# pmorenoz/HetMOGP

Hardware: AMD Instinct MI355X
Metric: ELBO-steps/sec (one step = ELBO + all parameter gradients) (higher is better)
Workload: dtype f64

## Files before the change

__graft_entry__.py:

```python
import os
import subprocess
import sys

ROOT = os.path.dirname(os.path.abspath(__file__))
CSRC = os.path.join(ROOT, "hetmogp_amd", "csrc")


def build():
    jobs = str(min(8, os.cpu_count() or 1))
    subprocess.run(["make", "-C", CSRC, "-j", jobs], check=True)
    probes = os.path.join(ROOT, "tools", "probes")
    os.makedirs(os.path.join(probes, "build"), exist_ok=True)
    for name in ("probe_mfma", "probe_coissue", "probe_gemm8", "probe_gemm16", "probe_gemm_abl", "probe_i8"):
        r = subprocess.run(["/opt/rocm/bin/hipcc", "--offload-arch=gfx950", "-O3", "-Wno-unused-value",
                            os.path.join(probes, name + ".hip"), "-o", os.path.join(probes, "build", name)], check=False)
        if r.returncode != 0:
            print("build(): diagnostic probe %s did not compile (not part of libhetmogp_hip.so)" % name, file=sys.stderr)
    if ROOT not in sys.path:
        sys.path.insert(0, ROOT)
    import hetmogp_amd
    from hetmogp_amd import _lib
    assert os.path.exists(_lib.LIB_PATH)


def smoke():
    if ROOT not in sys.path:
        sys.path.insert(0, ROOT)
    import numpy as np
    from hetmogp_amd.engine import Engine
    from hetmogp_amd.synthetic import make_case
    from oracle import svmogp_oracle as so

    specs = [("Gaussian", {"sigma": 0.5}), ("Bernoulli", {}), ("Poisson", {}), ("Gamma", {})]
    for M, N in ((64, 2000), (128, 20000)):
        prm, X, Y = make_case(specs, [N] * 4, M=M, Q=3, P=1, seed=7)
        prob = so.make_problem(specs, 3, M, 1)
        want = so.elbo_grad_fused(prm, prob, X, Y)
        e = Engine(specs, 3, M, 1, device=0)
        e.set_data(X, Y)
        out = e.elbo_grad(**prm)
        worst = 0.0
        for k in ("elbo", "g_m_u", "g_L_u", "g_variance", "g_lengthscale", "g_W", "g_kappa", "g_Z"):
            a, b = np.asarray(out[k], float), np.asarray(want[k], float)
            err = float(np.max(np.abs(a - b)) / (np.max(np.abs(b)) + 1e-300))
            worst = max(worst, err)
            assert err < 1e-8, (M, k, err)
        ms, _ = e.timings()
        print("smoke OK (M=%d, N_t=%d): ELBO %.6f (oracle %.6f), worst relative error %.2e, %.2f ms on device" %
              (M, N, out["elbo"], want["elbo"], worst, ms["total"]))
        e.close()
    g = np.load(os.path.join(ROOT, "tests", "golden", "lad_h_mix_M128_ladder.npz"))
    prm, prob, X, Y, bs = so.load_case(g)
    e = Engine(prob["specs"], prob["Q"], prob["M"], prob["P"], device=0, strict_qf=True)
    e.set_data(X, Y)
    out = e.elbo_grad(batch_scale=bs, **prm)
    assert out["rungs"] == [int(r) for r in g["rungs"]], out["rungs"]
    worst = 0.0
    for k in ("elbo", "g_m_u", "g_L_u", "g_variance", "g_lengthscale", "g_W", "g_kappa", "g_Z"):
        a, b = np.asarray(out[k], float).ravel(), np.asarray(g[k], float).ravel()
        ex = float(np.max(np.abs(a - b) / (1e-5 * np.abs(b) + 1e-9 * np.max(np.abs(b)))))
        worst = max(worst, ex)
        assert ex <= 1.0, ("strict mode vs reference run", k, ex)
    print("smoke OK (strict q(f), M=128, jitter rung %s as in the reference run): worst element-wise excess over 1e-5 criterion %.3f" %
          (out["rungs"], worst))
    from hetmogp_amd import _lib
    oe = e.elbo_grad(batch_scale=bs, group_mask=_lib.GROUP_QU, **prm)
    worst_e = 0.0
    for k in ("elbo", "g_m_u", "g_L_u"):
        a, b = np.asarray(oe[k], float).ravel(), np.asarray(g[k], float).ravel()
        ex = float(np.max(np.abs(a - b) / (1e-5 * np.abs(b) + 1e-9 * np.max(np.abs(b)))))
        worst_e = max(worst_e, ex)
        assert ex <= 1.0, ("strict E-step (one-solve form) vs reference run", k, ex)
    print("smoke OK (strict E-step, one-solve form): worst element-wise excess %.3f" % worst_e)
    e.close()


if __name__ == "__main__":
    build()
    if len(sys.argv) > 1 and sys.argv[1] == "smoke":
        smoke()
```

hetmogp_amd/csrc/gemm_rowpass.hip:

```cpp
#include <cstdlib>

#include "common.h"

namespace {

constexpr int BM = 128, BN = 128, BK = 16, W = 8, NT = W * 64;
constexpr int KM_LD = 144, RM_LD = 18, TILE_DOUBLES = BK * KM_LD;
constexpr int NB = 2, WN = 32, NWN = 4;

struct Tile {
  double a[2][TILE_DOUBLES];
  double b[2][TILE_DOUBLES];
};

__device__ __forceinline__ int diag_wm(int w) { return (0x4B >> w) & 1; }
__device__ __forceinline__ int diag_wn(int w) { return (0x7E84 >> (2 * w)) & 3; }

template <int ROLE, bool FOLD = false>
__device__ __forceinline__ void rowpass_tile(const GemmArgs& g, int tiles_n, int ti, int tj, int split, Tile& lds, double* epi_a,
                                             int* hwinfo = nullptr) {
  const int batch = blockIdx.z;
  const int M = g.M, N = g.N, K = g.K;
  const int i0 = ti * BM, j0 = tj * BN;
  if (i0 >= M || j0 >= N) return;
  int wlo = 0;
  if (ROLE == 1 && g.b_tri > 0) wlo = j0;
  const int ksteps = (K - wlo + BK - 1) / BK;
  const int per = (ksteps + g.ksplit - 1) / g.ksplit;
  const int kbeg = wlo + split * per * BK;
  const int kend = min(K, kbeg + per * BK);

  const double* __restrict__ A = g.A + (long long)batch * g.sA;
  const double* __restrict__ B = g.B + (long long)batch * g.sB;
  const double* __restrict__ S = (ROLE == 2) ? g.kscale + (long long)batch * g.sS : nullptr;
  double* __restrict__ C = g.C + (long long)batch * g.sC + (long long)split * g.sSplit;
  double* fs_part = (ROLE == 1 && g.fs_part) ? g.fs_part + (long long)batch * g.fs_sPart : nullptr;

  const int t = threadIdx.x, lane = t & 63, w = __builtin_amdgcn_readfirstlane(t >> 6);
  const int lr = lane & 15, lk = lane >> 4;
  int wm = w >> 2, wn = w & 3;
  if (FOLD && w >= 4) wn = 3 - wn;
  const int klive = FOLD ? j0 + 32 * wn : 0;
  unsigned sub = 0xFFu;
  const bool diag = ROLE == 2 && ti == tj && g.lower_only;
  if (diag && hwinfo) {
    if (lane == 0) {
      const unsigned hw = __builtin_amdgcn_s_getreg(4 | (0 << 6) | (31 << 11));
      hwinfo[w] = (int)((hw >> 4) & 3u);
      if (w == 0) hwinfo[8] = (int)((hw >> 1) & 1u);
    }
  }
  constexpr bool SWAP = (ROLE == 1);
  const int blr = SWAP ? 4 * (lr & 3) + (lr >> 2) : lr;

  f64x4 acc[4][NB];
#pragma unroll
  for (int a = 0; a < 4; ++a)
#pragma unroll
    for (int b = 0; b < NB; ++b) acc[a][b] = f64x4{0.0, 0.0, 0.0, 0.0};

  const int ar = t >> 2, ak = (t & 3) * 4, bk = t >> 5, bc = (t & 31) * 2;
  const double* pa;
  const double* pb;
  if (ROLE == 1) {
    pa = A + (long long)min(i0 + ar, M - 1) * g.lda + ak;
    pb = B + (long long)bk * g.ldb + j0 + bc;
  } else {
    pa = A + i0 + bc;
    pb = B + j0 + bc;
  }
  double ra[4], rb[4], ks = 1.0;
  auto load = [&](int k0) {
    if (ROLE == 1) {
      const f64x2 x0 = *reinterpret_cast<const f64x2*>(pa + k0), x1 = *reinterpret_cast<const f64x2*>(pa + k0 + 2);
      ra[0] = x0.x, ra[1] = x0.y, ra[2] = x1.x, ra[3] = x1.y;
      const double* q = pb + (long long)k0 * g.ldb;
      const f64x2 y0 = *reinterpret_cast<const f64x2*>(q), y1 = *reinterpret_cast<const f64x2*>(q + 64);
      rb[0] = y0.x, rb[1] = y0.y, rb[2] = y1.x, rb[3] = y1.y;
    } else {
      const int row = k0 + bk;
      const long long off = (long long)min(row, K - 1) * g.lda;
      const f64x2 x0 = *reinterpret_cast<const f64x2*>(pa + off), x1 = *reinterpret_cast<const f64x2*>(pa + off + 64);
      ra[0] = x0.x, ra[1] = x0.y, ra[2] = x1.x, ra[3] = x1.y;
      const f64x2 y0 = *reinterpret_cast<const f64x2*>(pb + off), y1 = *reinterpret_cast<const f64x2*>(pb + off + 64);
      rb[0] = y0.x, rb[1] = y0.y, rb[2] = y1.x, rb[3] = y1.y;
      ks = (row < kend) ? S[row] : 0.0;
    }
  };
  auto stage = [&](int buf) {
    if (ROLE == 1) {
      double* sa = &lds.a[buf][ar * RM_LD + ak];
      *reinterpret_cast<f64x2*>(sa) = f64x2{ra[0], ra[1]};
      *reinterpret_cast<f64x2*>(sa + 2) = f64x2{ra[2], ra[3]};
    } else {
      double* sa = &lds.a[buf][bk * KM_LD + bc];
      *reinterpret_cast<f64x2*>(sa) = f64x2{ra[0], ra[1]};
      *reinterpret_cast<f64x2*>(sa + 64) = f64x2{ra[2], ra[3]};
#pragma unroll
      for (int i = 0; i < 4; ++i) rb[i] *= ks;
    }
    double* sb = &lds.b[buf][bk * KM_LD + bc];
    *reinterpret_cast<f64x2*>(sb) = f64x2{rb[0], rb[1]};
    *reinterpret_cast<f64x2*>(sb + 64) = f64x2{rb[2], rb[3]};
  };
  double fa[2][4], fb[2][NB];
  auto frag = [&](int buf, int kk, int s) {
    const double* fpa = (ROLE == 1) ? &lds.a[buf][(wm * 64 + lr) * RM_LD + kk * 4 + lk] : &lds.a[buf][(kk * 4 + lk) * KM_LD + wm * 64 + lr];
    const double* fpb = &lds.b[buf][(kk * 4 + lk) * KM_LD + wn * WN + blr];
#pragma unroll
    for (int i = 0; i < 4; ++i) fa[s][i] = fpa[i * 16 * (ROLE == 1 ? RM_LD : 1)];
#pragma unroll
    for (int i = 0; i < NB; ++i) fb[s][i] = fpb[i * 16];
  };
  auto mm8 = [&](int s) {
#pragma unroll
    for (int a = 0; a < 4; ++a)
#pragma unroll
      for (int b = 0; b < NB; ++b) {
        if (ROLE == 2 && !((sub >> (a * NB + b)) & 1u)) continue;
        acc[a][b] = SWAP ? __builtin_amdgcn_mfma_f64_16x16x4f64(fb[s][b], fa[s][a], acc[a][b], 0, 0, 0)
                         : __builtin_amdgcn_mfma_f64_16x16x4f64(fa[s][a], fb[s][b], acc[a][b], 0, 0, 0);
      }
  };

  int cur = 0;
  if (kbeg < kend) {
    load(kbeg);
    stage(0);
    if (kbeg + BK < kend) load(kbeg + BK);
  }
  __syncthreads();
  if (diag) {
    int role = w;
    if (hwinfo) {
      bool ok = true;
      unsigned seen = 0;
#pragma unroll
      for (int i = 0; i < 4; ++i) {
        ok = ok && hwinfo[i] == hwinfo[i + 4];
        seen |= 1u << hwinfo[i];
      }
      if (ok && seen == 0xFu) role = ((hwinfo[w] + 2 * hwinfo[8]) & 3) + (w & 4);
    }
    role = __builtin_amdgcn_readfirstlane(role);
    wm = diag_wm(role), wn = diag_wn(role);
    sub = 0;
#pragma unroll
    for (int a = 0; a < 4; ++a)
#pragma unroll
      for (int b = 0; b < NB; ++b)
        if (wn * NB + b <= wm * 4 + a) sub |= 1u << (a * NB + b);
  }
  const bool live = ROLE == 1 || sub != 0;
  if (ROLE == 2) {
    for (int k0 = kbeg; k0 < kend; k0 += BK) {
      if (k0 + BK < kend) stage(cur ^ 1);
      if (k0 + 2 * BK < kend) load(k0 + 2 * BK);
      if (live) {
#pragma unroll
        for (int kk = 0; kk < BK / 4; ++kk) {
          frag(cur, kk, 0);
          mm8(0);
        }
      }
      __syncthreads();
      cur ^= 1;
    }
  }
  if (ROLE == 1 && kbeg < kend && (!FOLD || kbeg >= klive)) frag(0, 0, 0);
#define HM_SB __builtin_amdgcn_sched_barrier(0)
  for (int k0 = kbeg; ROLE == 1 && k0 < kend; k0 += BK) {
    const bool more = k0 + BK < kend;
    const bool lv = !FOLD || k0 >= klive;
    if (lv) {
      frag(cur, 1, 1);
      HM_SB;
      mm8(0);
      HM_SB;
    }
    if (more) stage(cur ^ 1);
    if (k0 + 2 * BK < kend) load(k0 + 2 * BK);
    HM_SB;
    if (lv) {
      frag(cur, 2, 0);
      HM_SB;
      mm8(1);
      HM_SB;
      frag(cur, 3, 1);
      HM_SB;
      mm8(0);
      HM_SB;
    }
    __syncthreads();
    if (more && (!FOLD || k0 + BK >= klive)) frag(cur ^ 1, 0, 0);
    if (lv) {
      HM_SB;
      mm8(1);
      HM_SB;
    }
    cur ^= 1;
  }
#undef HM_SB

  if (ROLE == 1 && fs_part && g.fs_sq) {
#pragma unroll
    for (int a = 0; a < 4; ++a) {
      double sq = 0.0;
#pragma unroll
      for (int b = 0; b < NB; ++b)
#pragma unroll
        for (int r = 0; r < 4; ++r) sq = fma(acc[a][b][r], acc[a][b][r], sq);
      sq += __shfl_xor(sq, 16, 64);
      sq += __shfl_xor(sq, 32, 64);
      const int rl = wm * 64 + a * 16 + lr;
      if (lk == 0 && i0 + rl < M) fs_part[((long long)NWN * tiles_n + NWN * tj + wn) * M + (i0 + rl)] = sq;
    }
    if (!g.store_c) return;
  } else if (ROLE == 1 && fs_part) {
    constexpr int NCH = 2 * NB, WSTAGE = 2 * NCH * 128;
    double* flat = &lds.a[0][0];
    double* stg = flat + w * WSTAGE;
    static_assert(W * WSTAGE <= 4 * TILE_DOUBLES, "epilogue scratch fits the tile buffers");
    const int colq = j0 + wn * WN + 4 * lk;
    const double* __restrict__ Ke = g.fs_k ? g.fs_k + (long long)batch * g.sA : A;
    auto issue = [&](int a) {
      const int grow = min(i0 + wm * 64 + a * 16 + lr, M - 1);
      const double* src = Ke + (long long)grow * g.lda + colq;
      double* dst = stg + (a & 1) * (NCH * 128);
#pragma unroll
      for (int c = 0; c < NCH; ++c)
        __builtin_amdgcn_global_load_lds((const void __attribute__((address_space(1)))*)(src + (c >> 1) * 16 + (c & 1) * 2),
                                         (void __attribute__((address_space(3)))*)(dst + c * 128), 16, 0, 0);
    };
    issue(0);
    issue(1);
    if (t < 128) epi_a[t] = g.fs_a[(long long)batch * g.fs_sA + j0 + t];
    __syncthreads();
#pragma unroll
    for (int a = 0; a < 4; ++a) {
      if (a < 3) asm volatile("s_waitcnt vmcnt(4)" ::: "memory");
      else asm volatile("s_waitcnt vmcnt(0)" ::: "memory");
      const int rl = wm * 64 + a * 16 + lr;
      double sp = 0.0, sc = 0.0;
#pragma unroll
      for (int b = 0; b < NB; ++b) {
        const int cl = wn * WN + b * 16 + 4 * lk;
        const double* kp = stg + (a & 1) * (NCH * 128) + (2 * b) * 128 + 2 * lane;
        const f64x2 k01 = *reinterpret_cast<const f64x2*>(kp), k23 = *reinterpret_cast<const f64x2*>(kp + 128);
        const double kv[4] = {k01.x, k01.y, k23.x, k23.y};
        const f64x2 a01 = *reinterpret_cast<const f64x2*>(epi_a + cl), a23 = *reinterpret_cast<const f64x2*>(epi_a + cl + 2);
        const double av[4] = {a01.x, a01.y, a23.x, a23.y};
#pragma unroll
        for (int r = 0; r < 4; ++r) {
          sp += kv[r] * av[r];
          sc += acc[a][b][r] * kv[r];
        }
      }
#pragma unroll
      for (int o = 16; o <= 32; o <<= 1) {
        sp += __shfl_xor(sp, o, 64);
        sc += __shfl_xor(sc, o, 64);
      }
      if (lk == 0 && i0 + rl < M) {
        double* o = fs_part + ((long long)(NWN * tj + wn)) * M + (i0 + rl);
        const long long ss = (long long)NWN * tiles_n * M;
        o[0] = sp, o[ss] = sc;
      }
      if (a < 2) {
        asm volatile("" ::: "memory");
        issue(a + 2);
      }
    }
    if (!g.store_c) return;
  }
  if (SWAP) {
#pragma unroll
    for (int a = 0; a < 4; ++a) {
      const int row = i0 + wm * 64 + a * 16 + lr;
      if (row >= M) continue;
      double* crow = C + (long long)row * g.ldc + j0 + wn * WN + 4 * lk;
      if (g.c_sub) {
        const double* srow = g.c_src ? g.c_src + (long long)batch * g.sC + (long long)row * g.ldc + j0 + wn * WN + 4 * lk : crow;
#pragma unroll
        for (int b = 0; b < NB; ++b) {
          const f64x2 c01 = *reinterpret_cast<const f64x2*>(srow + b * 16), c23 = *reinterpret_cast<const f64x2*>(srow + b * 16 + 2);
          *reinterpret_cast<f64x2*>(crow + b * 16) = f64x2{c01.x - acc[a][b][0], c01.y - acc[a][b][1]};
          *reinterpret_cast<f64x2*>(crow + b * 16 + 2) = f64x2{c23.x - acc[a][b][2], c23.y - acc[a][b][3]};
        }
        continue;
      }
#pragma unroll
      for (int b = 0; b < NB; ++b) {
        *reinterpret_cast<f64x2*>(crow + b * 16) = f64x2{acc[a][b][0], acc[a][b][1]};
        *reinterpret_cast<f64x2*>(crow + b * 16 + 2) = f64x2{acc[a][b][2], acc[a][b][3]};
      }
    }
    return;
  }
#pragma unroll
  for (int a = 0; a < 4; ++a)
#pragma unroll
    for (int r = 0; r < 4; ++r) {
      double* crow = C + (long long)(i0 + wm * 64 + a * 16 + 4 * r + lk) * g.ldc + j0 + wn * WN + lr;
#pragma unroll
      for (int b = 0; b < NB; ++b)
        if ((sub >> (a * NB + b)) & 1u) crow[b * 16] = acc[a][b][r];
    }
}

template <int ROLE, bool PAIR>
__device__ __forceinline__ void rowpass_block(const GemmArgs& g, int tiles_n, int ntiles, Tile& lds, double* epi_a,
                                              int* hwinfo = nullptr) {

  int v = blockIdx.x, split = 0;
  int ti, tj;
  if (ROLE == 2 && g.lower_only) {
    const int T = tiles_n, noff = T * (T - 1) / 2, ks8 = (g.ksplit > 1) ? ((g.ksplit + 7) / 8) * 8 : 1, gx1 = noff * ks8;
    if (v < gx1) {
      int u = v;
      if (g.ksplit > 1) {
        const int xcd = v & 7, idx = v >> 3;
        split = (idx / noff) * 8 + xcd;
        u = idx % noff;
      }
      ti = (int)((sqrt(8.0 * (double)u + 1.0) + 1.0) * 0.5);
      while (ti * (ti + 1) / 2 <= u) ++ti;
      while (ti * (ti - 1) / 2 > u) --ti;
      tj = u - ti * (ti - 1) / 2;
    } else {
      const int u = v - gx1;
      split = u / T;
      ti = tj = u - split * T;
    }
    if (split >= g.ksplit) return;
  } else {
    if (g.ksplit > 1) {
      const int xcd = v & 7, idx = v >> 3;
      split = (idx / ntiles) * 8 + xcd;
      v = idx % ntiles;
      if (split >= g.ksplit) return;
    } else if ((ntiles & 7) == 0) {
      const int cpx = ntiles >> 3;
      v = (v & 7) * cpx + (v >> 3);
    }
    const int tcols = PAIR ? tiles_n / 2 : tiles_n;
    ti = v / tcols;
    tj = v - ti * tcols;
  }
  rowpass_tile<ROLE, PAIR>(g, tiles_n, ti, tj, split, lds, epi_a, hwinfo);
  if (PAIR) {
    __syncthreads();
    rowpass_tile<ROLE, PAIR>(g, tiles_n, ti, tiles_n - 1 - tj, split, lds, epi_a);
  }
}

template <int ROLE>
__global__ __launch_bounds__(NT, 4) void rowpass_gemm_kernel(GemmArgs g, int tiles_n, int ntiles) {
  __shared__ __attribute__((aligned(16))) Tile lds;
  __shared__ __attribute__((aligned(16))) double epi_a[ROLE == 1 ? 128 : 2];
  __shared__ int hwinfo[ROLE == 2 ? 16 : 1];
  rowpass_block<ROLE, false>(g, tiles_n, ntiles, lds, epi_a, ROLE == 2 ? hwinfo : nullptr);
}
__global__ __launch_bounds__(NT, 4) void rowpass_fold_pair_kernel(GemmArgs g, int tiles_n, int ntiles) {
  __shared__ __attribute__((aligned(16))) Tile lds;
  __shared__ __attribute__((aligned(16))) double epi_a[128];
  rowpass_block<1, true>(g, tiles_n, ntiles, lds, epi_a);
}

bool aligned16(const void* p) { return (((uintptr_t)p) & 15) == 0; }

}

bool gemm_rowpass_eligible(const GemmArgs& g) {
  const bool sub = g.role == 1 && g.alpha == -1.0 && g.beta == 1.0 && !g.fs_part && g.b_tri == 0 && g.store_c;
  if (g.nouter != 1 || (!sub && (g.alpha != 1.0 || g.beta != 0.0)) || g.win || g.M_last || g.N_last || g.K_last || g.a_tri) return false;
  if ((g.lda & 1) || (g.ldb & 1) || (g.ldc & 1) || !aligned16(g.A) || !aligned16(g.B) || !aligned16(g.C)) return false;
  if (g.c_src && (!sub || !aligned16(g.c_src))) return false;
  if (g.fs_k && (g.role != 1 || !g.fs_part || g.fs_sq || !aligned16(g.fs_k))) return false;
  if ((g.sA & 1) || (g.sB & 1) || (g.sC & 1) || (g.sSplit & 1)) return false;
  if (g.role == 1)
    return !g.a_kmajor && g.b_kmajor && !g.lower_only && g.ksplit == 1 && !g.kscale && g.b_tri >= 0 && (g.N % BN) == 0 &&
           (g.K % BK) == 0 && (g.K == g.N || sub) && g.K >= BK && g.M >= 1;
  if (g.role == 2)
    return g.a_kmajor && g.b_kmajor && g.kscale && g.b_tri == 0 && g.M == g.N && (g.N % BN) == 0 &&
           g.lda == g.ldb && g.K >= 1;
  return false;
}

void launch_gemm_rowpass(const GemmArgs& g_in, hipStream_t stream) {
  GemmArgs g = g_in;
  g.c_sub = (g.role == 1 && g.alpha == -1.0 && g.beta == 1.0) ? 1 : 0;
  const int tiles_m = (g.M + BM - 1) / BM, tiles_n = (g.N + BN - 1) / BN;
  const int ntiles = g.lower_only ? tiles_m * (tiles_m + 1) / 2 : tiles_m * tiles_n;
  const int gx = (g.ksplit > 1) ? ntiles * ((g.ksplit + 7) / 8) * 8 : ntiles;
  dim3 grid(gx, 1, g.nbatch);
  if (g.role == 1) {
    const int pair = (g.b_tri > 0 && g.ksplit == 1 && tiles_n >= 2 && (tiles_n & 1) == 0) ? 1 : 0;
    if (pair) {
      grid.x = tiles_m * (tiles_n / 2);
      hipLaunchKernelGGL(rowpass_fold_pair_kernel, grid, dim3(NT), 0, stream, g, tiles_n, (int)grid.x);
    } else {
      hipLaunchKernelGGL((rowpass_gemm_kernel<1>), grid, dim3(NT), 0, stream, g, tiles_n, ntiles);
    }
  } else {
    hipLaunchKernelGGL((rowpass_gemm_kernel<2>), grid, dim3(NT), 0, stream, g, tiles_n, ntiles);
  }
}

int launch_gemm_rowpass_or_general(const GemmArgs& g, hipStream_t stream) {
  const bool eligible = gemm_rowpass_eligible(g);
  if ((g.fs_sq || g.fs_k) && !eligible)
    throw HipError{hipErrorInvalidValue, "fs_sq / fs_k are features of the specialised forward kernel only", __FILE__, __LINE__};
  if (eligible) {
    launch_gemm_rowpass(g, stream);
    return NWN;
  }
  if (g.role == 1 && (g.alpha != 1.0 || g.beta != 0.0)) {
    GemmArgs h = g;
    h.role = 0;
    launch_gemm_f64(h, stream);
    return 2;
  }
  launch_gemm_f64(g, stream);
  return 2;
}
```

Before: 8.386.

## Load B fragments directly from global via buffer loads in forward rowpass GEMM

Adds a B-direct variant of the forward (role 1) rowpass GEMM. B fragments are fetched straight from global memory into registers with raw buffer loads and a two-slot ring, while only A is staged through LDS at BK=32 with a new padded layout. This removes LDS traffic and barriers for B and halves the number of k-step syncs. The variant is selected when K is a multiple of 32, there is no subtract epilogue, no triangular B, and the buffer range fits in 32 bits; otherwise the old staged kernel runs. It risks global-load latency on the MFMA critical path and less reuse of B across waves.

```diff
diff --git a/__graft_entry__.py b/__graft_entry__.py
--- a/__graft_entry__.py
+++ b/__graft_entry__.py
@@ -11,7 +11,7 @@
     subprocess.run(["make", "-C", CSRC, "-j", jobs], check=True)
     probes = os.path.join(ROOT, "tools", "probes")
     os.makedirs(os.path.join(probes, "build"), exist_ok=True)
-    for name in ("probe_mfma", "probe_coissue", "probe_gemm8", "probe_gemm16", "probe_gemm_abl", "probe_i8"):
+    for name in ("probe_mfma", "probe_coissue", "probe_gemm8", "probe_gemm16", "probe_gemm_abl", "probe_gemm_bdirect", "probe_i8"):
         r = subprocess.run(["/opt/rocm/bin/hipcc", "--offload-arch=gfx950", "-O3", "-Wno-unused-value",
                             os.path.join(probes, name + ".hip"), "-o", os.path.join(probes, "build", name)], check=False)
         if r.returncode != 0:
diff --git a/hetmogp_amd/csrc/gemm_rowpass.hip b/hetmogp_amd/csrc/gemm_rowpass.hip
--- a/hetmogp_amd/csrc/gemm_rowpass.hip
+++ b/hetmogp_amd/csrc/gemm_rowpass.hip
@@ -7,6 +7,7 @@
 constexpr int BM = 128, BN = 128, BK = 16, W = 8, NT = W * 64;
 constexpr int KM_LD = 144, RM_LD = 18, TILE_DOUBLES = BK * KM_LD;
 constexpr int NB = 2, WN = 32, NWN = 4;
+constexpr int BK32 = 32, A32_LD = 34, BD_D = 2;
 
 struct Tile {
   double a[2][TILE_DOUBLES];
@@ -16,7 +17,7 @@
 __device__ __forceinline__ int diag_wm(int w) { return (0x4B >> w) & 1; }
 __device__ __forceinline__ int diag_wn(int w) { return (0x7E84 >> (2 * w)) & 3; }
 
-template <int ROLE, bool FOLD = false>
+template <int ROLE, bool FOLD = false, bool BD = false>
 __device__ __forceinline__ void rowpass_tile(const GemmArgs& g, int tiles_n, int ti, int tj, int split, Tile& lds, double* epi_a,
                                              int* hwinfo = nullptr) {
   const int batch = blockIdx.z;
@@ -123,13 +124,91 @@
       }
   };
 
+  if constexpr (BD) {
+    static_assert(ROLE == 1 && !FOLD, "B direct: the plain forward only");
+    constexpr int KS = BK32 / 4, NA = BK32 / 4;
+    static_assert(KS % BD_D == 0, "static ring slots");
+    static_assert(2 * BM * A32_LD <= 4 * TILE_DOUBLES, "A image at BK = 32 fits the tile buffers");
+    double* const img = &lds.a[0][0];
+    const int ar32 = t >> 2, ak32 = (t & 3) * 4;
+    const double* pa32 = A + (long long)min(i0 + ar32, M - 1) * g.lda + ak32;
+    double r32[NA];
+    auto load32 = [&](int k0) {
+      k0 = min(k0, kend - BK32);
+#pragma unroll
+      for (int i = 0; i < NA / 2; ++i) {
+        const f64x2 x = *reinterpret_cast<const f64x2*>(pa32 + k0 + (i >> 1) * 16 + (i & 1) * 2);
+        r32[2 * i] = x.x, r32[2 * i + 1] = x.y;
+      }
+    };
+    auto stage32 = [&](int buf) {
+      double* sa = img + buf * (BM * A32_LD) + ar32 * A32_LD + ak32;
+#pragma unroll
+      for (int i = 0; i < NA / 2; ++i) *reinterpret_cast<f64x2*>(sa + (i >> 1) * 16 + (i & 1) * 2) = f64x2{r32[2 * i], r32[2 * i + 1]};
+    };
+    const __amdgpu_buffer_rsrc_t brs = __builtin_amdgcn_make_buffer_rsrc(
+        const_cast<double*>(B), 0, (int)(sizeof(double) * ((long long)(K - 1) * g.ldb + N)), 0x00020000);
+    const int bvo = (int)sizeof(double) * (lk * g.ldb + j0 + wn * WN + blr);
+    double gb[BD_D][NB];
+    auto bload = [&](int k, int slot) {
+      const int so = __builtin_amdgcn_readfirstlane(min(k, kend - 4) * g.ldb * (int)sizeof(double));
+#pragma unroll
+      for (int b = 0; b < NB; ++b)
+        gb[slot][b] = __builtin_bit_cast(double, __builtin_amdgcn_raw_buffer_load_b64(brs, bvo + b * 16 * (int)sizeof(double), so, 0));
+    };
+    double ga[2][4];
+    auto frag32 = [&](int buf, int kk, int s) {
+      const double* fpa = img + buf * (BM * A32_LD) + (wm * 64 + lr) * A32_LD + kk * 4 + lk;
+#pragma unroll
+      for (int i = 0; i < 4; ++i) ga[s][i] = fpa[i * 16 * A32_LD];
+    };
+    auto mm32 = [&](int s, int slot) {
+#pragma unroll
+      for (int a = 0; a < 4; ++a)
+#pragma unroll
+        for (int b = 0; b < NB; ++b) acc[a][b] = __builtin_amdgcn_mfma_f64_16x16x4f64(gb[slot][b], ga[s][a], acc[a][b], 0, 0, 0);
+    };
+    int cur = 0;
+    if (kbeg < kend) {
+      load32(kbeg);
+      stage32(0);
+      load32(kbeg + BK32);
+#pragma unroll
+      for (int d = 0; d < BD_D; ++d) bload(kbeg + 4 * d, d);
+    }
+    __syncthreads();
+    if (kbeg < kend) frag32(0, 0, 0);
+    for (int k0 = kbeg; k0 < kend; k0 += BK32) {
+      const bool more = k0 + BK32 < kend;
+#pragma unroll
+      for (int kk = 0; kk < KS; ++kk) {
+        if (kk < KS - 1) {
+          frag32(cur, kk + 1, (kk + 1) & 1);
+        } else {
+          __syncthreads();
+          if (more) frag32(cur ^ 1, 0, 0);
+        }
+        __builtin_amdgcn_sched_barrier(0);
+        mm32(kk & 1, kk % BD_D);
+        __builtin_amdgcn_sched_barrier(0);
+        bload(k0 + 4 * (kk + BD_D), kk % BD_D);
+        if (kk == 0) {
+          if (more) stage32(cur ^ 1);
+          load32(k0 + 2 * BK32);
+        }
+        __builtin_amdgcn_sched_barrier(0);
+      }
+      cur ^= 1;
+    }
+  }
+
   int cur = 0;
-  if (kbeg < kend) {
+  if (!BD && kbeg < kend) {
     load(kbeg);
     stage(0);
     if (kbeg + BK < kend) load(kbeg + BK);
   }
-  __syncthreads();
+  if (!BD) __syncthreads();
   if (diag) {
     int role = w;
     if (hwinfo) {
@@ -167,9 +246,9 @@
       cur ^= 1;
     }
   }
-  if (ROLE == 1 && kbeg < kend && (!FOLD || kbeg >= klive)) frag(0, 0, 0);
+  if (ROLE == 1 && !BD && kbeg < kend && (!FOLD || kbeg >= klive)) frag(0, 0, 0);
 #define HM_SB __builtin_amdgcn_sched_barrier(0)
-  for (int k0 = kbeg; ROLE == 1 && k0 < kend; k0 += BK) {
+  for (int k0 = kbeg; ROLE == 1 && !BD && k0 < kend; k0 += BK) {
     const bool more = k0 + BK < kend;
     const bool lv = !FOLD || k0 >= klive;
     if (lv) {
@@ -308,7 +387,7 @@
     }
 }
 
-template <int ROLE, bool PAIR>
+template <int ROLE, bool PAIR, bool BD = false>
 __device__ __forceinline__ void rowpass_block(const GemmArgs& g, int tiles_n, int ntiles, Tile& lds, double* epi_a,
                                               int* hwinfo = nullptr) {
 
@@ -347,7 +426,7 @@
     ti = v / tcols;
     tj = v - ti * tcols;
   }
-  rowpass_tile<ROLE, PAIR>(g, tiles_n, ti, tj, split, lds, epi_a, hwinfo);
+  rowpass_tile<ROLE, PAIR, BD>(g, tiles_n, ti, tj, split, lds, epi_a, hwinfo);
   if (PAIR) {
     __syncthreads();
     rowpass_tile<ROLE, PAIR>(g, tiles_n, ti, tiles_n - 1 - tj, split, lds, epi_a);
@@ -359,7 +438,12 @@
   __shared__ __attribute__((aligned(16))) Tile lds;
   __shared__ __attribute__((aligned(16))) double epi_a[ROLE == 1 ? 128 : 2];
   __shared__ int hwinfo[ROLE == 2 ? 16 : 1];
-  rowpass_block<ROLE, false>(g, tiles_n, ntiles, lds, epi_a, ROLE == 2 ? hwinfo : nullptr);
+  rowpass_block<ROLE, false, ROLE == 1>(g, tiles_n, ntiles, lds, epi_a, ROLE == 2 ? hwinfo : nullptr);
+}
+__global__ __launch_bounds__(NT, 4) void rowpass_fwd_staged_kernel(GemmArgs g, int tiles_n, int ntiles) {
+  __shared__ __attribute__((aligned(16))) Tile lds;
+  __shared__ __attribute__((aligned(16))) double epi_a[128];
+  rowpass_block<1, false>(g, tiles_n, ntiles, lds, epi_a);
 }
 __global__ __launch_bounds__(NT, 4) void rowpass_fold_pair_kernel(GemmArgs g, int tiles_n, int ntiles) {
   __shared__ __attribute__((aligned(16))) Tile lds;
@@ -399,8 +483,10 @@
     if (pair) {
       grid.x = tiles_m * (tiles_n / 2);
       hipLaunchKernelGGL(rowpass_fold_pair_kernel, grid, dim3(NT), 0, stream, g, tiles_n, (int)grid.x);
+    } else if (!g.c_sub && g.b_tri == 0 && (g.K % BK32) == 0 && ((long long)(g.K - 1) * g.ldb + g.N) * (long long)sizeof(double) <= 0x7FFFFFFFLL) {
+      hipLaunchKernelGGL((rowpass_gemm_kernel<1>), grid, dim3(NT), 0, stream, g, tiles_n, ntiles);
     } else {
-      hipLaunchKernelGGL((rowpass_gemm_kernel<1>), grid, dim3(NT), 0, stream, g, tiles_n, ntiles);
+      hipLaunchKernelGGL(rowpass_fwd_staged_kernel, grid, dim3(NT), 0, stream, g, tiles_n, ntiles);
     }
   } else {
     hipLaunchKernelGGL((rowpass_gemm_kernel<2>), grid, dim3(NT), 0, stream, g, tiles_n, ntiles);
```

Result: faster. 8.568 (median of 6 runs) (+2.2%).
